# adamkewley/opensim-moco

Measured on AMD Instinct MI355X. Metric: NLP eval_g+eval_jac_g calls/sec (gait10dof18musc), higher is better.
Workload: dtype f64; 1 GPU; MocoTrack gait10dof18musc DGF rigid tendon (configs[2]); mesh_intervals=200, grid_points=401, n=26468, m=20800, nnz_jac=1920800, transcription=hermite-simpson, fd=forward, mode=separate, calls=asynchronous (device pointers, torch stream), parallelism=single

## Files before the change

### opensim-moco_amd/csrc/core.hpp

```cpp
#pragma once
#include <hip/hip_runtime.h>

#include <algorithm>
#include <cmath>
#include <cstdarg>
#include <cstdio>
#include <cstdlib>
#include <cstring>
#include <memory>
#include <string>
#include <type_traits>
#include <vector>

#include "../../include/mocohip.h"
#include "dae_device.hpp"

using namespace mh;

constexpr size_t kMaxLds = 160 * 1024;

typedef __attribute__((address_space(3))) double lds_double;
typedef __attribute__((address_space(3))) int lds_int;
__device__ __forceinline__ lds_double* lds(double* p) { return (lds_double*)p; }

// ... 572 lines not shown
    double* __restrict__ pf;
    const int* __restrict__ tab;
    int nslots;
    int nlc;
    int nl;
    int nq;
    int k0, kshift;
    __device__ __forceinline__ const int* slot(int npc) const { return tab; }
    __device__ __forceinline__ const int* chain(int npc) const { return tab + 2 * npc; }
    __device__ __forceinline__ const int* lane(int npc) const { return tab + 2 * npc + 2 * nslots; }
    __device__ __forceinline__ const int* coord(int npc) const { return lane(npc) + nq; }
    __device__ __forceinline__ const int* bodies(int npc) const { return coord(npc) + nlc; }
    __device__ __forceinline__ long at(int npc, int k, int ln, int e) const {
        return ((long)((k - k0) >> kshift) * nl + ln) * npc + e;
    }
};

struct PathEqs {
    int npc;
    const mh_path_equation* __restrict__ eq;
    const mh_table* __restrict__ tabs;
    const double* __restrict__ brk;
    const double* __restrict__ coef;
    const double* __restrict__ grid;
    FrameDist F;
};

struct EndpointEqs {
    int nep, nnz, W;
    const mh_endpoint_equation* __restrict__ eq;
    const TplEntry* __restrict__ tpl;
};

enum : uint32_t {
    CT_OFF = 0xFFFFFu,
    CT_RAW = 1u << 26,
    CT_GEN = 1u << 27,
    CT_PATH = 1u << 28
};
__device__ __host__ __forceinline__ uint32_t ct_word(uint32_t off, uint32_t coef, uint32_t base) {
    return off | (coef << 20) | (base << 23);
}

__device__ __forceinline__ double div_rn(double a, double b, double y) {
    double q = a * y;
    double r = __builtin_fma(-q, b, a);
    q = __builtin_fma(r, y, q);
    r = __builtin_fma(-q, b, a);
    q = __builtin_fma(r, y, q);
    const double m = __builtin_fabs(a);
    if (!(m >= 0x1p-900 && m <= 0x1p+900) && m != 0.0 && m == m) q = a / b;
    return m == 0.0 ? a * y : q;
}

struct Interval {
    int scheme;
    int interp;
    int ib;
    int rpi;
    int nnz_int;
    int nres;
    int nacc;
    int oaux;
    __device__ __forceinline__ int rout(int r) const { return r < nacc ? r : oaux + (r - nacc); }
    int N;
    int nnz_tail;
    int ntail;
    int npe;
    int nkr;
    int okc;
    PathEqs P;
    EndpointEqs E;
    double* gh;
    double* vh;
    int dbg_stop;
    int pf;
    int qfuse;
    int xcd;
    int dbase;
    uint32_t smagic, sstride, sbase;
    int qdiv;
    const uint32_t* ovl;
    int ov_ne[2], ov_nl[2];
    __device__ __forceinline__ uint32_t base_of(uint32_t w, uint32_t nyall) const {
        const uint32_t off = w & CT_OFF;
        const bool lane = !(w & (CT_GEN | CT_PATH)) && off < nyall;
        return lane ? __umulhi(off, smagic) * sstride + sbase : 0u;
    }
    __device__ __forceinline__ int rows(int i) const { return rpi + (i == N - 1 ? ntail : 0); }
    __device__ __forceinline__ int entries(int i) const { return nnz_int + (i == N - 1 ? nnz_tail : 0); }
};

__device__ __forceinline__ double path_bound(const PathEqs& P, const mh_path_equation& E, double t) {
#pragma clang fp contract(off)
    if (E.table < 0) return E.value;
    const mh_table T = P.tabs[E.table];
    const double* br = P.brk + T.break_begin;
    int s;
    if (t <= br[0]) s = 0;
    else if (t >= br[T.nseg]) s = T.nseg - 1;
    else {
        int lo = 0, hi = T.nseg;
        while (hi - lo > 1) {
            const int mid = (lo + hi) >> 1;
            if (t < br[mid]) hi = mid; else lo = mid;
        }
        s = lo;
    }
    const double* cf = P.coef + T.coef_begin + ((long)s * T.ncol + E.column) * (T.degree + 1);
    const double dt = t - br[s];
    double v = cf[T.degree];
    for (int k = T.degree - 1; k >= 0; --k) v = v * dt + cf[k];
    return v;
}
__device__ __forceinline__ double path_value(const PathEqs& P, int e, double t, double control) {
    const mh_path_equation E = P.eq[e];
    return control - path_bound(P, E, t);
}
__device__ __forceinline__ double path_quot(const PathEqs& P, const Lanes& Ln, int NS, int e, int k,
        double t, double control, int dir) {
#pragma clang fp contract(off)
    const mh_path_equation E = P.eq[e];
    if (dir >= 2 && dir != 2 + NS + E.index) return 0.0;
    const double h = Ln.h;
    double tp = t, tm = t, cp = control, cm = control;
    if (dir < 2) {
        const double g = P.grid[k];
        const double seed = dir == 0 ? 1.0 - g : g;
        tp = t + h * seed;
        tm = t - h * seed;
    } else {
        cp = control + h;
        cm = control - h;
    }
    if (Ln.fd == MH_FD_CENTRAL)
        return ((cp - path_bound(P, E, tp)) - (cm - path_bound(P, E, tm))) / (2.0 * h);
    const double v0 = control - path_bound(P, E, t);
    if (Ln.fd == MH_FD_FORWARD) return ((cp - path_bound(P, E, tp)) - v0) / h;
    return (v0 - (cm - path_bound(P, E, tm))) / h;
}

__device__ __forceinline__ double frame_quot(const PathEqs& P, const Lanes& Ln, int e, int k, int dir) {
#pragma clang fp contract(off)
    const FrameDist& F = P.F;
    if (dir < 2 || dir >= 2 + F.nq) return 0.0;
    const int l = F.lane(P.npc)[dir - 2];
    if (l < 0) return 0.0;
    const double h = Ln.h;
    const double v1 = F.pf[F.at(P.npc, k, 1 + l, e)];
    if (Ln.fd == MH_FD_CENTRAL) return (v1 - F.pf[F.at(P.npc, k, 1 + F.nlc + l, e)]) / (2.0 * h);
    const double v0 = F.pf[F.at(P.npc, k, 0, e)];
    if (Ln.fd == MH_FD_FORWARD) return (v1 - v0) / h;
    return (v0 - v1) / h;
}
template <class YV>
__device__ __forceinline__ double path_row(const PathEqs& P, const YV& Y, int e, int k) {
    const mh_path_equation E = P.eq[e];
    if (E.kind != MH_PATH_CONTROL_BOUND) return P.F.pf[P.F.at(P.npc, k, 0, e)];
    return path_value(P, e, Y.t(k), Y.xc(k, E.index));
}
template <class YV>
__device__ __forceinline__ double path_jac(const PathEqs& P, const Lanes& Ln, int NS, const YV& Y, int e, int k,
        int dir) {
    const mh_path_equation E = P.eq[e];
    if (E.kind != MH_PATH_CONTROL_BOUND) return frame_quot(P, Ln, e, k, dir);
    return path_quot(P, Ln, NS, e, k, Y.t(k), Y.xc(k, E.index), dir);
// ... 186 lines not shown
        if (dir >= 2) {
            v = 0.0 - C.h8 * (dxdot(L, Ln, Y, ki, s, dir) - dxdot(L, Ln, Y, kp, s, dir));
            break;
        }
        const double fi = xdot_at(L, Ln, x, Y, ki, s), fp = xdot_at(L, Ln, x, Y, kp, s);
        v = (dir == 0 ? C.g8 : -C.g8) * (fi - fp) -
            C.h8 * (dxdot(L, Ln, Y, ki, s, dir) - dxdot(L, Ln, Y, kp, s, dir));
        break;
    }
    case T_SIMP_T: {
        const int ki = k_first, km = k_first + 1, kp = k_first + 2;
        if (dir >= 2) {
            v = 0.0 - C.h6 * (dxdot(L, Ln, Y, kp, s, dir) + 4.0 * dxdot(L, Ln, Y, km, s, dir) +
                              dxdot(L, Ln, Y, ki, s, dir));
            break;
        }
        const double fi = xdot_at(L, Ln, x, Y, ki, s), fm = xdot_at(L, Ln, x, Y, km, s),
                     fp = xdot_at(L, Ln, x, Y, kp, s);
        v = (dir == 0 ? C.g6 : -C.g6) * (fp + 4.0 * fm + fi) -
            C.h6 * (dxdot(L, Ln, Y, kp, s, dir) + 4.0 * dxdot(L, Ln, Y, km, s, dir) +
                    dxdot(L, Ln, Y, ki, s, dir));
        break;
    }
    case T_HERM_X: {
        const int k = k_first + T.pt;
        const bool ident = dir == 2 + s;
        if (T.pt == 1) { v = ident ? 1.0 : 0.0; break; }
        if (ident) v += -0.5;
        const double dv = dxdot(L, Ln, Y, k, s, dir);
        v += (T.pt == 0 ? -C.h8 : C.h8) * dv;
        break;
    }
    case T_SIMP_X: {
        const int k = k_first + T.pt;
        const bool ident = dir == 2 + s;
        const double dv = dxdot(L, Ln, Y, k, s, dir);
        if (T.pt == 2) { if (ident) v += 1.0; v += -C.h6 * dv; }
        else if (T.pt == 0) { if (ident) v += -1.0; v += -C.h6 * dv; }
        else v += -C.h6 * 4.0 * dv;
        break;
    }
    case T_INTERP:
        v = T.pt == 1 ? 1.0 : -0.5;
        break;
    case T_RES:
        v = dout(Ln, Y, k_first + T.pt, s, dir);
        break;
    case T_PATH:
        if constexpr (WITH_PATH) {
            const int k = k_first + T.pt;
            v = path_jac(P, Ln, L.NS, Y, s, k, dir);
        }
        break;
    case T_TRAP_T: {
        const int ki = k_first, kp = k_first + 1;
        if (dir >= 2) {
            v = 0.0 - C.hh * (dxdot(L, Ln, Y, kp, s, dir) + dxdot(L, Ln, Y, ki, s, dir));
            break;
        }
        const double fi = xdot_at(L, Ln, x, Y, ki, s), fp = xdot_at(L, Ln, x, Y, kp, s);
        v = (dir == 0 ? C.gh : -C.gh) * (fp + fi) -
            C.hh * (dxdot(L, Ln, Y, kp, s, dir) + dxdot(L, Ln, Y, ki, s, dir));
        break;
    }
    case T_TRAP_X: {
        const int k = k_first + T.pt;
        const bool ident = dir == 2 + s;
        const double dv = dxdot(L, Ln, Y, k, s, dir);
        if (T.pt == 1) { if (ident) v += 1.0; v += -C.hh * dv; }
        else { if (ident) v += -1.0; v += -C.hh * dv; }
        break;
    }
    }
    return v;
}

__device__ __forceinline__ void interval_span(const Interval& I, int i, int& k_first, int& k_last) {
    k_first = grid_of(I, i, 0);
    k_last = k_first + (I.scheme == MH_HERMITE_SIMPSON ? 2 : 1);
}

constexpr int IV_UNROLL = 4;
constexpr int IV_PF = 12;
constexpr int CT_CONST = 4;
constexpr int CT_NCONST = 12;

template <class D, bool GM, bool BASE = false, bool SLDS = false, bool OV = false>
__device__ __forceinline__ void interval_body(const DevModel& M, const Src& S, const Lanes& Ln, const Tasks& TK,
        const Layout& L, const Interval& I, const TplEntry* __restrict__ tpl, const uint32_t* __restrict__ ctpl,
        const int* __restrict__ ctgen, int nctgen,
        const double* __restrict__ T, const double* __restrict__ H, double* __restrict__ g,
        double* __restrict__ values, int il) {
    extern __shared__ double smem[];
    if constexpr (BASE) values = nullptr;
    const int i = I.ib + il;
    int k_first, k_last;
    interval_span(I, i, k_first, k_last);
    const int npts = k_last - k_first + 1;
    const int nt = TK.tdoubles, nh = TK.nmass * D::NST;
    const int ny = D::NO * Ln.stride;
    double* sY = smem;
    double* sTimes = sY + npts * ny;
    double* sK = sTimes + CT_CONST;
    double* sT = sK + CT_NCONST;
    double* sH = sT + (GM ? 0 : npts * nt);
    double* sXs = sH + (GM ? 0 : npts * nh);
    double* sXc = sXs + npts * L.NS;
    double* sXd = sXc + npts * L.NC;
    double* sXm = sXd + npts * L.NDV;
    double* sXl = sXm + npts * L.NM;
    int* sSl = (int*)(sXl + L.NSL);
    const int kl0 = k_first - S.k0;
    if (I.dbg_stop == 7) return;
    if constexpr (BASE && GM) {
        if ((int)threadIdx.x < npts) {
            const int p = threadIdx.x;
            double t;
            const LaneIn<D> in = lane_input<D>(S, Ln, kl0 + p, Ln.base, t);
            sTimes[p] = t;
            const TaskLoadBase<D, const double*> TL{T + (long)(kl0 + p) * nt, H + (long)(kl0 + p) * nh};
            D::combine(M, t, in, TL, LdsOut{lds(sY + p * ny + Ln.base), Ln.stride});
        }
    }
    if (!GM && nt > 0) stage_lds<16>(sT, T + (long)kl0 * nt, npts * nt);
    if (!GM && nh > 0) stage_lds<8>(sH, H + (long)kl0 * nh, npts * nh);
    stage_lds<1>(sXs, S.x + 2 + (long)k_first * L.NS, npts * L.NS);
    if (L.NC > 0) stage_lds<1>(sXc, S.x + 2 + (long)L.NS * L.G + (long)k_first * L.NC, npts * L.NC);
    if (L.NDV > 0)
        stage_lds<1>(sXd, S.x + L.DB + (long)k_first * L.NDV, npts * L.NDV);
    if (L.NM > 0) stage_lds<1>(sXm, S.x + L.XM + (long)k_first * L.NM, npts * L.NM);
    if (L.NSL > 0) stage_lds<1>(sXl, S.x + L.XL + (long)i * L.NSL, L.NSL);
    if constexpr (SLDS)
        for (int q = threadIdx.x; q < Ln.stride * D::NG; q += blockDim.x) sSl[q] = TK.jd[q];
    const double t0 = S.x[0], tf = S.x[1];
    if (threadIdx.x < 2) sK[threadIdx.x] = threadIdx.x ? 1.0 : 0.0;
    __syncthreads();
    if (I.dbg_stop == 1) return;
    using PartAll = std::integral_constant<int, 0>;
    using PartCopies = std::integral_constant<int, 1>;
    using PartSolved = std::integral_constant<int, 2>;
    auto combine_lane = [&](int p, int r, auto partc) {
        constexpr int PART = decltype(partc)::value;
        LaneInL<D> in{lds(sXs + p * L.NS), lds(sXc + p * L.NC), lds(sXd + p * L.NDV), -1, 0.0,
                      lds(sXm + p * L.NM), L.vc(k_first + p) ? lds(sXl) : nullptr};
        const double t = lane_time(Ln, S.grid[k_first + p], t0, tf, r, in.pi, in.step);
        if (PART != 2 && r == Ln.base) sTimes[p] = t;
        const LdsOut out{lds(sY + p * ny + r), Ln.stride};
        auto run = [&](const auto& TL) {
            if constexpr (PART == 1) D::combine_copies(M, t, in, TL, out);
            else if constexpr (PART == 2) D::combine_solved(M, t, in, TL, out);
            else D::combine(M, t, in, TL, out);
        };
        if constexpr (BASE) {
            const TaskLoadBase<D, const lds_double*> TL{lds(sT + p * nt), lds(sH + p * nh)};
            D::combine(M, t, in, TL, out);
        } else if constexpr (GM) {
            const TaskLoadGlobal<D> TL{T + (long)(kl0 + p) * nt, H + (long)(kl0 + p) * nh, TK.jd, r};
            D::combine(M, t, in, TL, out);
        } else if constexpr (SLDS) {
            const TaskLoadLds<D, const lds_int*> TL{lds(sT + p * nt), lds(sH + p * nh), (const lds_int*)sSl, r};
            run(TL);
        } else {
            const TaskLoadLds<D> TL{lds(sT + p * nt), lds(sH + p * nh), TK.jd, r};
            run(TL);
        }
    };
    if constexpr (OV && !BASE && !GM) {
        {
#pragma clang fp contract(off)
            const int B = blockDim.x, tid = threadIdx.x;
            const int nl = npts * Ln.stride;
            const int ncw = (nl + 63) >> 6;
            const int cp = tid / Ln.stride, cr = tid - cp * Ln.stride;
            if (tid < nl) combine_lane(cp, cr, PartCopies{});
            if (tid == B - 1) {
                int pi;
                double st;
                const double ta = lane_time(Ln, S.grid[k_first], t0, tf, Ln.base, pi, st);
                const double tb = lane_time(Ln, S.grid[k_last], t0, tf, Ln.base, pi, st);
                const IvC C0 = iv_const(tb - ta, S.grid[k_last] - S.grid[k_first]);
                sK[2] = 0.0; sK[3] = -C0.h8; sK[4] = C0.h8; sK[5] = -C0.h6; sK[6] = -C0.h6 * 4.0; sK[7] = -C0.hh;
                sK[8] = 0.0; sK[9] = -0.5; sK[10] = 1.0; sK[11] = -1.0;
            }
            __syncthreads();
            double* vi = values + (long)il * I.nnz_int;
            const lds_double* q0 = lds(sY);
            const lds_double* kc = lds(sK + 2);
            const lds_double* kb = lds(sK + 8);
            const int nyall = npts * ny;
            const double h1 = Ln.h, h2 = 2.0 * Ln.h;
            auto run_list = [&](auto fdc, const uint32_t* __restrict__ le, int cap, int n, int j0, int J) {
                constexpr int FD = decltype(fdc)::value;
                const uint32_t* __restrict__ lw = le + cap;
                const uint32_t* __restrict__ lb = lw + cap;
                auto value = [&](uint32_t wu, double q) {
                    const double coef = kc[(wu >> 20) & 7], base = kb[(wu >> 23) & 7];
                    return (wu & CT_RAW) ? q : base + coef * q;
                };
                auto qat = [&](uint32_t off, uint32_t boff) -> double {
                    const double y = q0[off];
                    const bool lane = (int)off < nyall;
                    const double ym = FD == MH_FD_CENTRAL ? q0[lane ? off + Ln.ND : off] : q0[boff];
                    const double qd = FD == MH_FD_CENTRAL ? (y - ym) / h2
                                    : FD == MH_FD_FORWARD ? (y - ym) / h1 : (ym - y) / h1;
                    return lane ? qd : y;
                };
                int j = j0;
                for (; j + (IV_UNROLL - 1) * J < n; j += IV_UNROLL * J) {
                    uint32_t e[IV_UNROLL], w[IV_UNROLL], wb[IV_UNROLL];
                    double q[IV_UNROLL];
#pragma unroll
                    for (int u = 0; u < IV_UNROLL; ++u) {
                        e[u] = le[j + u * J];
                        w[u] = lw[j + u * J];
                        wb[u] = lb[j + u * J];
                    }
#pragma unroll
                    for (int u = 0; u < IV_UNROLL; ++u) q[u] = qat(w[u] & CT_OFF, wb[u]);
#pragma unroll
                    for (int u = 0; u < IV_UNROLL; ++u) vi[e[u]] = value(w[u], q[u]);
                }
                for (; j < n; j += J) {
                    const uint32_t wu = lw[j];
                    vi[le[j]] = value(wu, qat(wu & CT_OFF, lb[j]));
                }
            };
            auto assemble = [&](const uint32_t* le, int cap, int n, int j0, int J) {
                if (Ln.fd == MH_FD_FORWARD) run_list(std::integral_constant<int, MH_FD_FORWARD>{}, le, cap, n, j0, J);
                else if (Ln.fd == MH_FD_BACKWARD)
                    run_list(std::integral_constant<int, MH_FD_BACKWARD>{}, le, cap, n, j0, J);
                else run_list(std::integral_constant<int, MH_FD_CENTRAL>{}, le, cap, n, j0, J);
            };
            const int last = i == I.N - 1;
            if ((tid >> 6) < ncw) {
                if (tid < nl) combine_lane(cp, cr, PartSolved{});
            } else if (I.dbg_stop != 2) {
                assemble(I.ovl, I.ov_ne[1], I.ov_ne[last], tid - ncw * 64, B - ncw * 64);
            }
            __syncthreads();
            if (I.dbg_stop == 2 || I.dbg_stop == 8) return;
            const YS YV{lds(sY), lds(sTimes), D::NO, Ln.stride, k_first, 0, lds(sXs), lds(sXc), L.NS, L.NC,
                        lds(sXd), L.NDV};
            auto g_rows = [&]() {
                if (!g) return;
                double* gi = g + (long)il * I.rpi;
                for (int r = tid; r < I.rows(i); r += B) gi[r] = defect_row(L, I, Ln, S.x, YV, i, r);
            };
            if (I.dbg_stop == 4) { g_rows(); return; }
            assemble(I.ovl + 3 * (long)I.ov_ne[1], I.ov_nl[1], I.ov_nl[last], tid, B);
            const IvC C = iv_const(YV.t(k_last) - YV.t(k_first), S.grid[k_last] - S.grid[k_first]);
            for (int j = tid; j < nctgen; j += B) {
                const int eg = ctgen[j];
                vi[eg] = jac_entry<false>(L, Ln, I.P, S.x, YV, tpl[eg], k_first, C);
            }
            if (I.npe > 0) {
                const int npe = I.npe;
                const int nw = last ? 2 * npe : npe;
                for (int w = tid; w < nw; w += B) {
                    const int ep = w < npe ? w : I.nnz_int + (w - npe);
                    vi[ep] = jac_entry<true>(L, Ln, I.P, S.x, YV, tpl[ep], k_first, C);
                }
            }
            g_rows();
            if (i == 0 && (I.gh || I.vh))
                endpoint_head(L, Ln, I.E, S.x, g ? I.gh : nullptr, I.vh, tid, B);
            return;
        }
    }
    if constexpr (BASE && GM) {
    } else if (BASE || Ln.stride == 1) {
        if ((int)threadIdx.x < npts) combine_lane((int)threadIdx.x, 0, PartAll{});
    } else {
        for (int w = threadIdx.x; w < npts * Ln.stride; w += blockDim.x) {
            const int p = w / Ln.stride, r = w - p * Ln.stride;
            combine_lane(p, r, PartAll{});
        }
    }
    const int ne_iv = values ? I.entries(i) : 0;
    uint32_t pw[IV_PF];
#pragma unroll
    for (int u = 0; u < IV_PF; ++u) {
        const int e = threadIdx.x + u * blockDim.x;
        pw[u] = I.pf && ctpl && e < ne_iv ? ctpl[e] : CT_GEN;
    }
    const uint32_t* __restrict__ cbase = ctpl ? ctpl + I.nnz_int + I.nnz_tail : nullptr;
    uint32_t pb[IV_PF];
#pragma unroll
    for (int u = 0; u < IV_PF; ++u) {
        const int e = threadIdx.x + u * blockDim.x;
        pb[u] = I.pf && ctpl && e < ne_iv ? cbase[e] : 0u;
    }
    int eg0 = -1;
    TplEntry tg0{};
    if (I.pf && ctpl && values && (int)threadIdx.x < nctgen) {
        eg0 = ctgen[threadIdx.x];
        tg0 = tpl[eg0];
    }
    __syncthreads();
    if (values && ctpl && threadIdx.x == 0) {
        const IvC C0 = iv_const(sTimes[npts - 1] - sTimes[0], S.grid[k_last] - S.grid[k_first]);
        sK[2] = 0.0; sK[3] = -C0.h8; sK[4] = C0.h8; sK[5] = -C0.h6; sK[6] = -C0.h6 * 4.0; sK[7] = -C0.hh;
        sK[8] = 0.0; sK[9] = -0.5; sK[10] = 1.0; sK[11] = -1.0;
    }
    if (I.dbg_stop == 2) return;
    const int quot = values && Ln.stride > 1 && !I.qfuse;
    if (quot) {
#pragma clang fp contract(off)
        const int wave = threadIdx.x >> 6, lane = threadIdx.x & 63, nwave = blockDim.x >> 6;
        const double h = Ln.h, h2 = 2.0 * Ln.h;
        for (int po = wave; po < npts * D::NO; po += nwave) {
            lds_double* y = lds(sY + po * Ln.stride);
            const double yb = y[Ln.base];
            for (int d = lane; d < Ln.ND; d += 64) {
                double q;
                if (Ln.fd == MH_FD_CENTRAL) q = (y[d] - y[Ln.ND + d]) / h2;
                else if (Ln.fd == MH_FD_FORWARD) q = (y[d] - yb) / h;
                else q = (yb - y[d]) / h;
                y[d] = q;
            }
        }
        __syncthreads();
    }
    const YS YV{lds(sY), lds(sTimes), D::NO, Ln.stride, k_first, quot, lds(sXs), lds(sXc), L.NS, L.NC,
                lds(sXd), L.NDV};
    if (I.dbg_stop == 3) return;
    if (I.dbg_stop >= 5 && values) {
        double* vi = values + (long)il * I.nnz_int;
        const int ne = I.entries(i);
        double acc = 0.0;
        for (int e = threadIdx.x; e < ne; e += blockDim.x) {
            if (I.dbg_stop == 5) vi[e] = 0.0;
            else {
// ... 673 lines not shown
    std::vector<int> fd_tab;
    size_t fd_lds = 0;
    std::vector<mh_goal> goals;
    std::vector<int32_t> gidx, gcol;
    std::vector<double> gw;
    int nep = 0, nnz_ep = 0;
    int NPAR = 0, NCOPY = 1;
    int64_t XP = 0;
    std::vector<mh_bounds> par_bounds;
    std::vector<mh_parameter_target> par_targets;
    mh_parameter_target* d_par_targets = nullptr;
    std::vector<DevModel> Mp;
    DevModel M0{};
    int* d_lane_main = nullptr;
    int n_lane_main = 0;
    int* d_par_lanes = nullptr;
    int nsprings = 0;
    std::vector<mh_endpoint_equation> ep;
    std::vector<TplEntry> eptpl;
    std::vector<uint8_t> sp_ep;
    EndpointEqs E{};
    double acc_lo = -1000.0, acc_hi = 1000.0;
    int ib = 0, ie = 0, k0 = 0, nk = 0;
    int fd = 0;
    double h = 1e-8;
    int size_class = 0;
    const struct Backend* be = nullptr;
    const struct GenEntry* gen = nullptr;
    Lanes lanes_jac{}, lanes_g{};
    uint64_t model_hash = 0;
    int64_t n = 0, m = 0, nnz = 0;
    std::vector<double> grid, quad;
    std::vector<TplEntry> tpl;
    std::vector<int> tpl_col_pt;
    std::vector<int64_t> tpl_col_off;
    std::vector<mh_variable_info> sinfo, cinfo;
    mh_bounds t_init{}, t_final{};
    int ngoals = 0;
    int device = 0;
    hipStream_t stream = nullptr;
    hipStream_t own_stream = nullptr;
    bool async = false;
    int iv_dbg_stop = 0;
    int iv_pf = 1;
    int iv_dbase = 0;
    std::vector<int> exc_xs;
    bool exc_redirected = false;
    bool exc_full = false;
    uint32_t iv_smagic = 0, iv_sstride = 1, iv_sbase = 0;
    int iv_qdiv = 0;
    int iv_xcd = 1;
    int iv_qfuse = 1;
    hipEvent_t ev[5] = {};
    static constexpr int kMaxD2hChunks = 16;
    int d2h_chunks = 1;
    hipStream_t copy_stream = nullptr;
    hipEvent_t ev_chunk[kMaxD2hChunks] = {};
    hipEvent_t ev_copied = nullptr;
    char* dmem = nullptr;
    DevModel M{};
    GoalSet GS{};
    double* d_quadp = nullptr;
    std::vector<double> quadp;
    double *d_x = nullptr, *d_grid = nullptr, *d_quad = nullptr, *d_times = nullptr, *d_Y = nullptr,
           *d_Yg = nullptr, *d_g = nullptr, *d_vals = nullptr, *d_C = nullptr, *d_grad = nullptr,
           *d_tpart = nullptr, *d_f = nullptr;
    TplEntry* d_tpl = nullptr;
    int* d_exc = nullptr;
    int* d_lane_map = nullptr;
    int n_exc_lanes = 0;
    int* d_exc_slot = nullptr;
    int* d_cmb_map = nullptr;
    int n_exc_gen = 0;
    int g_block = 4;
    bool g_lds = false;
    int g_lds_guard = 0;
    int* d_lds_status = nullptr;
    int groups_split = -1;
    int combine_mode = -1;
    uint32_t* d_ctpl = nullptr;
    std::vector<uint32_t> ctpl;
    int* d_ctgen = nullptr;
    int iv_overlap = 0;
    std::vector<uint32_t> ovl;
    uint32_t* d_ovl = nullptr;
    int ov_ne[2] = {0, 0}, ov_nl[2] = {0, 0};
    std::vector<int> ctgen;
    std::vector<int> rl_e;
    std::vector<uint32_t> rl_w;
    int rl_off[4] = {0, 0, 0, 0}, rl_tail[2] = {0, 0};
    int* d_rl_e = nullptr;
    uint32_t* d_rl_w = nullptr;
    double* d_xch = nullptr;
    double* d_ep = nullptr;
    bool has_marker = false;
    MarkerTrack MT{};
    std::vector<int> mt_tab;
    size_t mt_lds[2] = {0, 0};
    bool use_roles = false;
    int role_threads = 256;
    int iv_threads = 1024;
    int ivg_threads = 256;
    int csplit = 0;
    int ivg_base = 1;
    int ivg_gm = -1;
    int iv_slots_lds = 0;
    bool role_couple = true;
    bool use_ctpl = true;
    float timings[4] = {0, 0, 0, 0};
    TaskSet ts_jac, ts_g, ts_probe;
    bool krec_ok = false;
    KRecs krec_g{};
    double *d_T = nullptr, *d_H = nullptr;
    double *d_Tg = nullptr, *d_Hg = nullptr;
    hipStream_t aux_stream = nullptr;
    hipEvent_t ev_x = nullptr, ev_aux = nullptr;
    const double* x_last = nullptr;
    bool overlap = false;
    char* probe_mem = nullptr;
    double *d_pT = nullptr, *d_pH = nullptr;
    int probe_np = -1;
    struct GraphEntry { int kind; const void *x, *a, *b; hipGraphExec_t exec; };
    std::vector<GraphEntry> graphs;
    bool use_graphs = false;
    bool spin_wait = false;
    bool use_interval[2] = {false, false};
    int nsimd = 1024;
    bool asm_grid_stride = false;
    bool asm_ctpl = true;
    int asm_chunk_ct = 8192;
    bool quot = false;
    const Backend* be_lane = nullptr;
    bool g_lane = false;
    int yq[2] = {0, 0};
    bool timing = false;
    bool groups_timed = false;
    int jac_seeds = 0, nseeds = 0;
    int coloring_order = MH_COLORING_SMALLEST_LAST;
    std::vector<int32_t> seed_color;
    std::vector<int32_t> seed_col_off, seed_cols, seed_ent_off, seed_ents, seed_rows;
    int32_t *d_seed_cols = nullptr, *d_seed_ents = nullptr, *d_seed_rows = nullptr;
    double *d_xp = nullptr, *d_xm = nullptr, *d_gp = nullptr, *d_gm = nullptr;
};

inline Layout make_layout(const mh_ctx* c, int k0, int nk) {
    Layout L{c->NS, c->NC, c->TQ, c->NO, c->NI, c->G, k0, nk, c->NDV, c->NACC, c->SO,
             c->NM, c->NSL, c->OQC, 0, 0, 0};
    L.XM = 2 + (long)(c->NS + c->NC) * c->G;
    L.XL = L.XM + (long)c->NM * c->G;
    L.DB = L.XL + (long)c->NSL * c->N;
    return L;
}

inline Interval make_interval(const mh_ctx* c, double*& g, double*& v) {
    Interval I{c->scheme, c->interp, c->ib, c->rpi, c->nnz_int, c->NMB + c->NAR, c->NMB, c->NQ + c->NZ,
               c->N, c->nnz_tail, c->ntail, c->npe, c->NK, c->OKC, c->P, c->E, nullptr, nullptr, c->iv_dbg_stop, c->iv_pf, c->iv_qfuse,
               c->iv_xcd, c->iv_dbase, c->iv_smagic, c->iv_sstride, c->iv_sbase,
               c->iv_qdiv, c->d_ovl, {c->ov_ne[0], c->ov_ne[1]}, {c->ov_nl[0], c->ov_nl[1]}};
    if (c->ib == 0 && c->nep > 0) {
        I.gh = g;
        I.vh = v;
        if (g) g += c->nep;
        if (v) v += c->nnz_ep;
    }
    return I;
}

inline Src src_of(const mh_ctx* c, const double* x) {
    const Layout L = make_layout(c, c->k0, c->nk);
    return Src{x, c->d_grid, nullptr, c->G, c->k0, L.XM, L.XL, L.DB};
}

int probe_tasks(mh_ctx* c, const TaskInfo& ti, const Lanes& ln, int np);

struct mh_batch {
    std::vector<mh_ctx*> ctx;
    int B = 0;
    BatchItem* d_items = nullptr;
    bool gm = true;
    int waves = 3;
    int threads = 512;
};

struct Backend {
    const char* name;
    void (*eval)(mh_ctx*, const double* x, int mode, double* Y);
    void (*integrand)(mh_ctx*, const double* x);
    void (*grad)(mh_ctx*, const double* x);
    void (*probe)(mh_ctx*, int np, const double* in, double* out);
    double flops_per_eval;
    const TaskInfo* tasks;
    void (*interval)(mh_ctx*, const double* x, int mode, double* g, double* v, int i0, int i1);
    size_t (*interval_bytes)(const mh_ctx*, int mode);
    void (*lanes)(mh_ctx*, const double* x, double* Y);
    void (*batch)(mh_batch*, int mode, const BatchPtrs& P, int with_g, int with_v);
};

template <class D>
static void be_eval_lane(mh_ctx* c, const double* x, int mode, double* Y) {
    Layout L = make_layout(c, c->k0, c->nk);
    const Lanes& ln = mode ? c->lanes_jac : c->lanes_g;
    const long lanes = (long)c->nk * ln.stride;
    const bool exc = mode && c->d_exc && D::EXC_LANES;
    if (mode && c->NPAR > 0) {
        const long nm = (long)c->nk * c->n_lane_main;
        hipLaunchKernelGGL(k_eval<D>, dim3((unsigned)((nm + 63) / 64)), dim3(64), 0, c->stream, c->M, L, ln, x,
                c->d_grid, c->d_times, Y, c->d_lane_main, c->n_lane_main);
        if (exc)
            hipLaunchKernelGGL(k_exc_lanes<D>, dim3((unsigned)((lanes + 63) / 64)), dim3(64), 0, c->stream, c->M,
                    L, ln, x, Y, c->d_exc);
        for (int cp = 1; cp < c->NCOPY; ++cp)
            hipLaunchKernelGGL(k_eval<D>, dim3((unsigned)((c->nk + 63) / 64)), dim3(64), 0, c->stream, c->Mp[cp],
                    L, ln, x, c->d_grid, c->d_times, Y, c->d_par_lanes + (cp - 1), 1);
        return;
    }
    if (!exc) {
        const int tb = (mode == 0 && D::EXC_LANES) ? c->g_block : 64;
        if constexpr (D::EXC_LANES) {
            if (mode == 0 && c->g_lds) {
                const size_t slot = sizeof(typename D::W) + 2 * sizeof(double) * (size_t)c->g_lds_guard;
                const int tl = std::max(1, std::min({tb, 16, (int)(65536 / slot)}));
                const size_t lds = slot * (size_t)tl;
                hipLaunchKernelGGL(k_eval_lds<D>, dim3((unsigned)((lanes + tl - 1) / tl)), dim3(tl), lds,
                        c->stream, c->M, L, ln, x, c->d_grid, c->d_times, Y, c->g_lds_guard, c->d_lds_status);
                return;
            }
        }
        hipLaunchKernelGGL(k_eval<D>, dim3((unsigned)((lanes + tb - 1) / tb)), dim3(tb), 0, c->stream, c->M, L,
                ln, x, c->d_grid, c->d_times, Y, nullptr, 0);
        return;
    }
    const int nmap = ln.stride - c->n_exc_lanes;
    const long full = (long)c->nk * nmap;
    hipLaunchKernelGGL(k_eval<D>, dim3((unsigned)((full + 63) / 64)), dim3(64), 0, c->stream, c->M, L,
            ln, x, c->d_grid, c->d_times, Y, c->d_lane_map, nmap);
    hipLaunchKernelGGL(k_exc_lanes<D>, dim3((unsigned)((lanes + 63) / 64)), dim3(64), 0, c->stream, c->M,
            L, ln, x, Y, c->d_exc);
}
template <class D>
static bool split_groups(const mh_ctx* c) {
    static int decided = -1;
// ... 269 lines not shown
```

### opensim-moco_amd/csrc/mocohip.hip

```cpp
#include "core.hpp"

#include <cstdarg>
#include <limits>

static thread_local std::string g_err;
static int set_err(int code, const char* fmt, ...) {
    char buf[1024];
    va_list ap;
    va_start(ap, fmt);
    vsnprintf(buf, sizeof buf, fmt, ap);
    va_end(ap);
    g_err = buf;
    return code;
}
#define HIPCHK(expr)                                                              \
    do {                                                                          \
        hipError_t e_ = (expr);                                                   \
        if (e_ != hipSuccess)                                                     \
            return set_err(MH_ERR_HIP, "%s failed: %s", #expr, hipGetErrorString(e_)); \
    } while (0)

extern "C" int mh_abi_version(void) { return MH_ABI_VERSION; }
#ifndef MH_BUILD_ID
#define MH_BUILD_ID "unknown"
// ... 2303 lines not shown
        const char* eg = std::getenv("MOCOHIP_GRAPHS");
        c->use_graphs = eg && std::strcmp(eg, "1") == 0;
        const char* es = std::getenv("MOCOHIP_SPIN");
        c->spin_wait = es && std::strcmp(es, "1") == 0;
        const char* ei = std::getenv("MOCOHIP_INTERVAL");
        const bool allow = !(ei && std::strcmp(ei, "0") == 0);
        const char* ec = std::getenv("MOCOHIP_CTPL");
        c->use_ctpl = !(ec && std::strcmp(ec, "0") == 0);
        setup_assembly_variants(c.get());
        const char* er = std::getenv("MOCOHIP_ROLES");
        c->use_roles = er && std::strcmp(er, "1") == 0 && c->NM == 0;
        const char* et = std::getenv("MOCOHIP_ROLE_THREADS");
        if (et) c->role_threads = std::min(512, std::max(64, std::atoi(et) / 64 * 64));
        const char* eqf = std::getenv("MOCOHIP_IV_QFUSE");
        c->iv_qfuse = !(eqf && std::strcmp(eqf, "0") == 0);
        const char* eth = std::getenv("MOCOHIP_IV_THREADS");
        if (eth) c->iv_threads = std::min(1024, std::max(256, std::atoi(eth) / 64 * 64));
        const char* egt = std::getenv("MOCOHIP_IVG_THREADS");
        if (egt) c->ivg_threads = std::min(1024, std::max(64, std::atoi(egt) / 64 * 64));
        const char* eo = std::getenv("MOCOHIP_ROLE_COUPLE");
        c->role_couple = !(eo && std::strcmp(eo, "0") == 0);
        const char* ea = std::getenv("MOCOHIP_ASM");
        c->asm_grid_stride = ea && std::strcmp(ea, "gs") == 0;
        const char* eac = std::getenv("MOCOHIP_ASM_CTPL");
        c->asm_ctpl = !(eac && std::strcmp(eac, "0") == 0);
        if (const char* ech = std::getenv("MOCOHIP_ASM_CHUNK"))
            c->asm_chunk_ct = std::min(1 << 20, std::max(256, std::atoi(ech)));
        const char* ee = std::getenv("MOCOHIP_EVENTS");
        c->timing = ee && std::strcmp(ee, "1") == 0;
        const char* egl = std::getenv("MOCOHIP_G_LANE");
        c->g_lane = egl && std::strcmp(egl, "1") == 0;
        const char* eq = std::getenv("MOCOHIP_QUOT");
        c->quot = eq && std::strcmp(eq, "1") == 0;
        if (redirect_exc_words(c.get()) > 0) {
            setup_assembly_variants(c.get());
            HIPCHK(hipMemcpy(c->d_ctpl, c->ctpl.data(), sizeof(uint32_t) * c->ctpl.size(),
                    hipMemcpyHostToDevice));
        }
        if (o->sparsity_detection != MH_SPARSITY_NONE) {
            const size_t cap = c->tpl.size(), cap_ep = c->eptpl.size();
            int rc2 = detect_sparsity(c.get(), o);
            if (rc2) return rc2;
            c->tpl.clear();
            c->tpl_col_pt.clear();
            build_template(c.get());
            if (!path_entries_lead(c.get()) || c->tpl.size() > cap || c->eptpl.size() > cap_ep)
                return set_err(MH_ERR_INVALID, "internal: detected template layout");
            if (!c->eptpl.empty())
                HIPCHK(hipMemcpy((void*)c->E.tpl, c->eptpl.data(), sizeof(TplEntry) * c->eptpl.size(),
                        hipMemcpyHostToDevice));
            c->E.nnz = c->nnz_ep;
            c->nnz = c->nnz_ep + (int64_t)c->nnz_int * c->N + c->nnz_tail;
            if (!compile_template(c.get())) return set_err(MH_ERR_UNSUPPORTED, "Jacobian template does not compile");
            (void)redirect_exc_words(c.get());
            setup_assembly_variants(c.get());
            HIPCHK(hipMemcpy(c->d_tpl, c->tpl.data(), sizeof(TplEntry) * c->tpl.size(), hipMemcpyHostToDevice));
            HIPCHK(hipMemcpy(c->d_ctpl, c->ctpl.data(), sizeof(uint32_t) * c->ctpl.size(),
                    hipMemcpyHostToDevice));
            if (!c->ctgen.empty())
                HIPCHK(hipMemcpy(c->d_ctgen, c->ctgen.data(), sizeof(int) * c->ctgen.size(),
                        hipMemcpyHostToDevice));
            if (!c->rl_e.empty()) {
                HIPCHK(hipMemcpy(c->d_rl_e, c->rl_e.data(), sizeof(int) * c->rl_e.size(), hipMemcpyHostToDevice));
                HIPCHK(hipMemcpy(c->d_rl_w, c->rl_w.data(), sizeof(uint32_t) * c->rl_w.size(),
                        hipMemcpyHostToDevice));
            }
            c->P.npc = c->npc;
        }
        for (int mode = 0; mode < 2; ++mode)
            c->use_interval[mode] = allow && interval_fits(c.get(), mode);
        const char* eio = std::getenv("MOCOHIP_IV_OVERLAP");
        const int npts_ov = c->scheme == MH_HERMITE_SIMPSON ? 3 : 2;
        const int ncw = (npts_ov * c->lanes_jac.stride + 63) / 64;
        const int ds = c->iv_dbg_stop;
        if (!(eio && std::strcmp(eio, "0") == 0) && tib && c->use_interval[1] && c->use_ctpl && c->iv_qfuse &&
                !c->use_roles && c->lanes_jac.stride > 1 && c->iv_threads > 256 && c->iv_threads / 64 > ncw &&
                ds != 3 && ds != 5 &&
                ds != 6) {
            if (!build_overlap_lists(c.get(), *tib) || c->ovl.size() > ovl_cap)
                return set_err(MH_ERR_INVALID, "internal: k_interval's early entries read a solved output");
            if (!c->ovl.empty())
                HIPCHK(hipMemcpy(c->d_ovl, c->ovl.data(), sizeof(uint32_t) * c->ovl.size(), hipMemcpyHostToDevice));
            c->iv_overlap = 1;
        }
    }
    for (auto& e : c->ev) HIPCHK(hipEventCreate(&e));
    if (const char* ek = std::getenv("MOCOHIP_D2H_CHUNKS"))
        c->d2h_chunks = std::min(mh_ctx::kMaxD2hChunks, std::max(1, std::atoi(ek)));
    HIPCHK(hipStreamCreateWithFlags(&c->aux_stream, hipStreamNonBlocking));
    HIPCHK(hipEventCreateWithFlags(&c->ev_x, hipEventDisableTiming));
    HIPCHK(hipEventCreateWithFlags(&c->ev_aux, hipEventDisableTiming));
    if (const char* eov = std::getenv("MOCOHIP_OVERLAP")) c->overlap = std::strcmp(eov, "1") == 0;
    HIPCHK(hipStreamCreateWithFlags(&c->copy_stream, hipStreamNonBlocking));
    for (auto& e : c->ev_chunk) HIPCHK(hipEventCreateWithFlags(&e, hipEventDisableTiming));
    HIPCHK(hipEventCreateWithFlags(&c->ev_copied, hipEventDisableTiming));
    *out = c.release();
    return MH_OK;
}

extern "C" void mh_destroy(mh_ctx* c) {
    if (!c) return;
    (void)hipSetDevice(c->device);
    if (c->stream) (void)hipStreamSynchronize(c->stream);
    for (auto& e : c->ev)
        if (e) (void)hipEventDestroy(e);
    for (auto& e : c->ev_chunk)
        if (e) (void)hipEventDestroy(e);
    if (c->ev_copied) (void)hipEventDestroy(c->ev_copied);
    if (c->aux_stream) {
        (void)hipStreamSynchronize(c->aux_stream);
        (void)hipStreamDestroy(c->aux_stream);
    }
    if (c->ev_x) (void)hipEventDestroy(c->ev_x);
    if (c->ev_aux) (void)hipEventDestroy(c->ev_aux);
    if (c->copy_stream) {
        (void)hipStreamSynchronize(c->copy_stream);
        (void)hipStreamDestroy(c->copy_stream);
    }
    if (c->own_stream) {
        (void)hipStreamSynchronize(c->own_stream);
        (void)hipStreamDestroy(c->own_stream);
    }
    if (c->dmem) (void)hipFree(c->dmem);
    if (c->probe_mem) (void)hipFree(c->probe_mem);
    for (auto& e : c->graphs) (void)hipGraphExecDestroy(e.exec);
    delete c;
}

extern "C" int mh_get_nlp_info(const mh_ctx* c, mh_nlp_info* info) {
    if (!c || !info) return set_err(MH_ERR_INVALID, "null argument");
    std::memset(info, 0, sizeof *info);
    info->n = c->n;
    info->m = c->m;
    info->nnz_jac_g = c->nnz;
    info->nnz_h_lag = 0;
    info->num_grid_points = c->G;
    info->num_states = c->NS;
    info->num_controls = c->NC;
    info->row_begin = c->ib == 0 ? 0 : c->nep + (int64_t)c->ib * c->rpi;
    info->row_end = c->nep + (int64_t)c->ie * c->rpi + (c->ie == c->N ? c->ntail : 0);
    info->nnz_begin = c->ib == 0 ? 0 : c->nnz_ep + (int64_t)c->ib * c->nnz_int;
    info->nnz_end = c->nnz_ep + (int64_t)c->ie * c->nnz_int + (c->ie == c->N ? c->nnz_tail : 0);
    return MH_OK;
}

static mh_bounds clip(mh_bounds b, mh_bounds e) {
    mh_bounds r;
    r.lower = std::max(b.lower, e.lower);
    r.upper = std::min(b.upper, e.upper);
    return r;
}
static void put_bounds(mh_bounds b, double& lo, double& up) {
    if (!std::isnan(b.lower) && !std::isnan(b.upper)) { lo = b.lower; up = b.upper; }
    else { lo = -INFINITY; up = INFINITY; }
}

extern "C" int mh_get_bounds(const mh_ctx* c, double* xl, double* xu, double* gl, double* gu) {
    if (!c || !xl || !xu) return set_err(MH_ERR_INVALID, "null argument");
    put_bounds(c->t_init, xl[0], xu[0]);
    put_bounds(c->t_final, xl[1], xu[1]);
    auto fill = [&](const mh_variable_info& vi, auto col) {
        const mh_bounds ib = clip(vi.bounds, vi.initial), fb = clip(vi.bounds, vi.final);
        for (int k = 1; k < c->G - 1; ++k) put_bounds(vi.bounds, xl[col(k)], xu[col(k)]);
        put_bounds(ib, xl[col(0)], xu[col(0)]);
        put_bounds(fb, xl[col(c->G - 1)], xu[col(c->G - 1)]);
    };
// ... 1107 lines not shown
    if (flops_per_eval) *flops_per_eval = c->be->flops_per_eval;
    if (model_hash) *model_hash = c->model_hash;
    return MH_OK;
}

extern "C" int mh_get_nlp_info_for(const mh_problem* p, const mh_options* o, mh_nlp_info* info) {
    if (!p || !o || !info) return set_err(MH_ERR_INVALID, "null argument");
    std::unique_ptr<mh_ctx> c(new mh_ctx());
    std::vector<int> coord_body, act_state, ftn_state, mus_control;
    double tau_act, tau_deact;
    int rc = validate_and_layout(c.get(), p, o, coord_body, act_state, ftn_state, mus_control, tau_act,
            tau_deact);
    if (rc) return rc;
    FrameDist FD;
    MarkerTrack MT;
    if ((rc = kinematics_tables(c.get(), p->model, coord_body, FD, MT))) return rc;
    return mh_get_nlp_info(c.get(), info);
}

extern "C" int mh_backend_for(const mh_problem* p, const mh_options* o, char* name, int32_t name_len) {
    if (!p || !o || !name || name_len <= 0) return set_err(MH_ERR_INVALID, "bad argument");
    std::unique_ptr<mh_ctx> c(new mh_ctx());
    std::vector<int> coord_body, act_state, ftn_state, mus_control;
    double tau_act, tau_deact;
    int rc = validate_and_layout(c.get(), p, o, coord_body, act_state, ftn_state, mus_control, tau_act,
            tau_deact);
    if (rc) return rc;
    const Backend* be = select_backend(c.get(), p);
    std::strncpy(name, be->name, (size_t)name_len - 1);
    name[name_len - 1] = 0;
    return MH_OK;
}

extern "C" int mh_debug_interval_overlap(const mh_problem* p, const mh_options* o, int32_t* info8, uint32_t* words,
        uint32_t* bases, uint8_t* early, uint8_t* out_early, int64_t cap) {
    if (!p || !o || !info8) return set_err(MH_ERR_INVALID, "bad argument");
    std::unique_ptr<mh_ctx> c(new mh_ctx());
    std::vector<int> coord_body, act_state, ftn_state, mus_control;
    double tau_act, tau_deact;
    int rc = validate_and_layout(c.get(), p, o, coord_body, act_state, ftn_state, mus_control, tau_act,
            tau_deact);
    if (rc) return rc;
    const Backend* be = select_backend(c.get(), p);
    if (!compile_template(c.get())) return set_err(MH_ERR_UNSUPPORTED, "Jacobian template does not compile");
    const size_t nw = (size_t)c->nnz_int + (size_t)c->nnz_tail;
    const int ND = c->NI + 2 + c->NPAR;
    const int stride = c->fd == MH_FD_CENTRAL ? 2 * ND + 1 : ND + 1;
    const int npts = c->scheme == MH_HERMITE_SIMPSON ? 3 : 2;
    const int32_t info[8] = {(int32_t)nw, c->nnz_int, npts, c->NO, stride, ND, c->fd, stride - 1};
    std::copy(info, info + 8, info8);
    if (cap < (int64_t)nw || cap < c->NO) return MH_OK;
    if (!words || !bases || !early || !out_early) return set_err(MH_ERR_INVALID, "null argument");
    const TaskInfo* ti = be->tasks;
    for (int q = 0; q < c->NO; ++q) out_early[q] = ti && ti->no == c->NO ? ti->out_early[q] : 0;
    std::copy(c->ctpl.begin(), c->ctpl.begin() + nw, words);
    std::copy(c->ctpl.begin() + nw, c->ctpl.begin() + 2 * nw, bases);
    classify_overlap(c->ctpl.data(), nw, npts, c->NO, stride, ND, c->fd, ti && ti->no == c->NO ? ti->out_early : nullptr,
            early);
    return MH_OK;
}

extern "C" int mh_get_callback_sparsity(const mh_ctx* c, uint8_t* pattern, int64_t len) {
    if (!c || !pattern) return set_err(MH_ERR_INVALID, "null argument");
    const size_t W = 1 + (size_t)c->NI, nd = (size_t)c->NO * W, np = nd + (size_t)c->npc * W;
    const size_t need = np + (size_t)c->nep * 2 * W;
    if (len < (int64_t)need) return set_err(MH_ERR_INVALID, "pattern needs %zu bytes", need);
    for (size_t i = 0; i < need; ++i)
        pattern[i] = i < nd ? (c->sp.empty() ? 1 : c->sp[i])
                   : i < np ? (c->sp_pc.empty() ? 1 : c->sp_pc[i - nd])
                            : (c->sp_ep.empty() ? 1 : c->sp_ep[i - np]);
    return MH_OK;
}

extern "C" int mh_get_backend_flags(const mh_ctx* c, char* flags, int32_t len) {
    if (!c || !flags || len <= 0) return set_err(MH_ERR_INVALID, "bad argument");
    std::string f = c->be->tasks ? "tasks" : (std::strncmp(c->be->name, "generic", 7) == 0 ? "generic" : "lane");
    f += c->use_interval[1] ? " interval" : " split";
    if (c->use_interval[0]) f += c->ivg_base ? " interval-g base-slots" : " interval-g";
    if (c->krec_ok) f += " groups-kernarg";
    if (!c->use_ctpl) f += " no-ctpl";
    if (c->iv_dbase) f += " dbase";
    if (c->iv_qdiv) f += " qdiv";
    if (c->use_roles && c->use_interval[1]) f += " roles";
    if (c->iv_overlap && c->use_interval[1]) f += " iv-overlap";
    if (c->quot) f += " quot";
    if (c->asm_grid_stride) f += " asm-gs";
    if (c->d_exc) f += " exc-lanes";
    if (c->d_exc_slot)
        f += c->exc_redirected && c->use_ctpl && c->asm_ctpl && !c->asm_grid_stride ? " exc-fill adot-only"
                                                                                     : " exc-fill";
    if (c->g_lds && !c->be->tasks && std::strncmp(c->be->name, "generic", 7) == 0) {
        f += " g-lds";
        if (c->g_lds_guard) {
            int st = 0;
            if (hipMemcpyAsync(&st, c->d_lds_status, sizeof(int), hipMemcpyDeviceToHost, c->stream) != hipSuccess ||
                    hipStreamSynchronize(c->stream) != hipSuccess)
                return set_err(MH_ERR_HIP, "reading the LDS guard status failed");
            f += st ? " g-lds-guard-violated" : " g-lds-guard-intact";
        }
    }
    std::strncpy(flags, f.c_str(), (size_t)len - 1);
    flags[len - 1] = 0;
    return MH_OK;
}

extern "C" int mh_get_work(const mh_ctx* c, double* work4) {
    if (!c || !work4) return set_err(MH_ERR_INVALID, "null argument");
    const double lanes_jac = (double)c->nk * c->lanes_jac.stride, lanes_g = (double)c->nk;
    if (c->be->tasks) {
        work4[0] = c->ts_jac.flops;
        work4[1] = c->ts_g.flops;
        work4[2] = c->ts_jac.ntasks;
    } else {
        work4[0] = lanes_jac * c->be->flops_per_eval;
        work4[1] = lanes_g * c->be->flops_per_eval;
        work4[2] = 0.0;
    }
    work4[3] = lanes_jac;
    return MH_OK;
}

static const Backend* select_backend(mh_ctx* c, const mh_problem* p) {
    c->model_hash = model_hash(&p->model);
    const char* force = std::getenv("MOCOHIP_BACKEND");
    const bool generic = force && std::strcmp(force, "generic") == 0;
    const bool lane = force && std::strcmp(force, "lane") == 0;
    if (!generic && c->NPAR == 0 && c->nsprings == 0) {
        for (auto entry : kGeneratedModels) {
            const GenEntry& e = entry();
            if (e.implicit != (c->NMB > 0) || e.prescribed != (c->presc != 0)) continue;
            if (c->NKC && !c->presc && (e.kc_enforce != (c->enforce != 0) || e.kc_slacks != (c->NSL > 0)))
                continue;
            if (!e.match(p->model)) continue;
            c->gen = &e;
            c->be_lane = &e.lane;
            return lane ? &e.lane : &e.tasks;
        }
    }
    return &generic_backends()[c->size_class];
}
```

Measured before the change: 26300 calls/s.

## Software-pipeline overlap-list index loads in interval Jacobian assembly

Adds a pipelined assembly path for the overlapped interval kernel. Index triples for the early list are loaded before LDS staging. The next batch of indices is prefetched while the current batch is computed. Late-list indices are loaded ahead by the combine warps before the barrier, and the time-step constants are computed earlier. The aim is to hide global-memory latency on index fetches, at the cost of more registers (IvBatch copies) and added code complexity, with an env var to turn it off.

```diff
diff --git a/opensim-moco_amd/csrc/core.hpp b/opensim-moco_amd/csrc/core.hpp
--- a/opensim-moco_amd/csrc/core.hpp
+++ b/opensim-moco_amd/csrc/core.hpp
@@ -678,6 +678,7 @@
     int qdiv;
     const uint32_t* ovl;
     int ov_ne[2], ov_nl[2];
+    int pipe;
     __device__ __forceinline__ uint32_t base_of(uint32_t w, uint32_t nyall) const {
         const uint32_t off = w & CT_OFF;
         const bool lane = !(w & (CT_GEN | CT_PATH)) && off < nyall;
@@ -1030,6 +1031,14 @@
 
 constexpr int IV_UNROLL = 4;
 constexpr int IV_PF = 12;
+constexpr int IVP_BATCH = 1;
+constexpr int IVP_EARLY = 2;
+constexpr int IVP_LATE = 4;
+constexpr int IVP_CONST = 8;
+constexpr int IVP_DEFAULT = IVP_BATCH | IVP_EARLY | IVP_LATE | IVP_CONST;
+struct IvBatch {
+    uint32_t e[IV_UNROLL], w[IV_UNROLL], wb[IV_UNROLL];
+};
 constexpr int CT_CONST = 4;
 constexpr int CT_NCONST = 12;
 
@@ -1060,6 +1069,35 @@
     int* sSl = (int*)(sXl + L.NSL);
     const int kl0 = k_first - S.k0;
     if (I.dbg_stop == 7) return;
+    auto iv_load = [&](IvBatch& b, uint32_t off, int cap, int n, int j, int J) {
+#pragma unroll
+        for (int u = 0; u < IV_UNROLL; ++u) {
+            const int ju = j + u * J;
+            const bool ok = ju < n;
+            const uint32_t o = ok ? off + (uint32_t)ju : 0u, c = ok ? (uint32_t)cap : 0u;
+            b.e[u] = I.ovl[o];
+            b.w[u] = I.ovl[o + c];
+            b.wb[u] = I.ovl[o + 2u * c];
+        }
+    };
+    const int ivp = I.pipe;
+    IvBatch ovb;
+    if constexpr (OV && !BASE && !GM) {
+        const int B = blockDim.x, tid = threadIdx.x;
+        const int ncw = (npts * Ln.stride + 63) >> 6;
+        if ((ivp & IVP_EARLY) && (tid >> 6) >= ncw && I.dbg_stop != 2)
+            iv_load(ovb, 0u, I.ov_ne[1], I.ov_ne[i == I.N - 1], tid - ncw * 64, B - ncw * 64);
+        if ((ivp & IVP_CONST) && tid == B - 1) {
+#pragma clang fp contract(off)
+            int pi;
+            double st;
+            const double ta = lane_time(Ln, S.grid[k_first], S.x[0], S.x[1], Ln.base, pi, st);
+            const double tb = lane_time(Ln, S.grid[k_last], S.x[0], S.x[1], Ln.base, pi, st);
+            const IvC C0 = iv_const(tb - ta, S.grid[k_last] - S.grid[k_first]);
+            sK[2] = 0.0; sK[3] = -C0.h8; sK[4] = C0.h8; sK[5] = -C0.h6; sK[6] = -C0.h6 * 4.0; sK[7] = -C0.hh;
+            sK[8] = 0.0; sK[9] = -0.5; sK[10] = 1.0; sK[11] = -1.0;
+        }
+    }
     if constexpr (BASE && GM) {
         if ((int)threadIdx.x < npts) {
             const int p = threadIdx.x;
@@ -1121,7 +1159,7 @@
             const int ncw = (nl + 63) >> 6;
             const int cp = tid / Ln.stride, cr = tid - cp * Ln.stride;
             if (tid < nl) combine_lane(cp, cr, PartCopies{});
-            if (tid == B - 1) {
+            if (!(ivp & IVP_CONST) && tid == B - 1) {
                 int pi;
                 double st;
                 const double ta = lane_time(Ln, S.grid[k_first], t0, tf, Ln.base, pi, st);
@@ -1137,22 +1175,61 @@
             const lds_double* kb = lds(sK + 8);
             const int nyall = npts * ny;
             const double h1 = Ln.h, h2 = 2.0 * Ln.h;
+            auto value = [&](uint32_t wu, double q) {
+                const double coef = kc[(wu >> 20) & 7], base = kb[(wu >> 23) & 7];
+                return (wu & CT_RAW) ? q : base + coef * q;
+            };
+            auto quot_at = [&](auto fdc, uint32_t off, uint32_t boff) -> double {
+                constexpr int FD = decltype(fdc)::value;
+                const double y = q0[off];
+                const bool lane = (int)off < nyall;
+                const double ym = FD == MH_FD_CENTRAL ? q0[lane ? off + Ln.ND : off] : q0[boff];
+                const double qd = FD == MH_FD_CENTRAL ? (y - ym) / h2
+                                : FD == MH_FD_FORWARD ? (y - ym) / h1 : (ym - y) / h1;
+                return lane ? qd : y;
+            };
+            const int last = i == I.N - 1;
+            const uint32_t loff = 3u * (uint32_t)I.ov_ne[1];
+            const int ne = I.ov_ne[last], nla = I.ov_nl[last];
+            auto run_pipe = [&](auto fdc, IvBatch& cur, uint32_t off, int cap, int n, int j0, int J, bool then_late) {
+                for (int j = j0; j < n;) {
+                    const int jn = j + IV_UNROLL * J;
+                    const bool more = jn < n;
+                    IvBatch nxt = cur;
+                    if (then_late)
+                        iv_load(nxt, more ? off : loff, more ? cap : I.ov_nl[1], more ? n : nla, more ? jn : tid,
+                                more ? J : B);
+                    else if (more) iv_load(nxt, off, cap, n, jn, J);
+                    double q[IV_UNROLL];
+#pragma unroll
+                    for (int u = 0; u < IV_UNROLL; ++u) {
+                        const bool ok = j + u * J < n;
+                        q[u] = quot_at(fdc, ok ? cur.w[u] & CT_OFF : 0u, ok ? cur.wb[u] : 0u);
+                    }
+                    double v[IV_UNROLL];
+#pragma unroll
+                    for (int u = 0; u < IV_UNROLL; ++u) v[u] = value(j + u * J < n ? cur.w[u] : 0u, q[u]);
+#pragma unroll
+                    for (int u = 0; u < IV_UNROLL; ++u) asm volatile("" : "+v"(v[u]));
+#pragma unroll
+                    for (int u = 0; u < IV_UNROLL; ++u)
+                        if (j + u * J < n) vi[cur.e[u]] = v[u];
+                    cur = nxt;
+                    j = jn;
+                }
+                if (then_late && j0 >= n) iv_load(cur, loff, I.ov_nl[1], nla, tid, B);
+            };
+            auto assemble_pipe = [&](IvBatch& cur, uint32_t off, int cap, int n, int j0, int J, bool then_late) {
+                if (Ln.fd == MH_FD_FORWARD)
+                    run_pipe(std::integral_constant<int, MH_FD_FORWARD>{}, cur, off, cap, n, j0, J, then_late);
+                else if (Ln.fd == MH_FD_BACKWARD)
+                    run_pipe(std::integral_constant<int, MH_FD_BACKWARD>{}, cur, off, cap, n, j0, J, then_late);
+                else run_pipe(std::integral_constant<int, MH_FD_CENTRAL>{}, cur, off, cap, n, j0, J, then_late);
+            };
             auto run_list = [&](auto fdc, const uint32_t* __restrict__ le, int cap, int n, int j0, int J) {
-                constexpr int FD = decltype(fdc)::value;
                 const uint32_t* __restrict__ lw = le + cap;
                 const uint32_t* __restrict__ lb = lw + cap;
-                auto value = [&](uint32_t wu, double q) {
-                    const double coef = kc[(wu >> 20) & 7], base = kb[(wu >> 23) & 7];
-                    return (wu & CT_RAW) ? q : base + coef * q;
-                };
-                auto qat = [&](uint32_t off, uint32_t boff) -> double {
-                    const double y = q0[off];
-                    const bool lane = (int)off < nyall;
-                    const double ym = FD == MH_FD_CENTRAL ? q0[lane ? off + Ln.ND : off] : q0[boff];
-                    const double qd = FD == MH_FD_CENTRAL ? (y - ym) / h2
-                                    : FD == MH_FD_FORWARD ? (y - ym) / h1 : (ym - y) / h1;
-                    return lane ? qd : y;
-                };
+                auto qat = [&](uint32_t off, uint32_t boff) -> double { return quot_at(fdc, off, boff); };
                 int j = j0;
                 for (; j + (IV_UNROLL - 1) * J < n; j += IV_UNROLL * J) {
                     uint32_t e[IV_UNROLL], w[IV_UNROLL], wb[IV_UNROLL];
@@ -1179,11 +1256,20 @@
                     run_list(std::integral_constant<int, MH_FD_BACKWARD>{}, le, cap, n, j0, J);
                 else run_list(std::integral_constant<int, MH_FD_CENTRAL>{}, le, cap, n, j0, J);
             };
-            const int last = i == I.N - 1;
+            const bool batch = ivp & IVP_BATCH, late_ahead = batch && (ivp & IVP_LATE);
+            IvBatch ovt;
             if ((tid >> 6) < ncw) {
                 if (tid < nl) combine_lane(cp, cr, PartSolved{});
+                if (late_ahead && I.dbg_stop != 2) iv_load(ovt, loff, I.ov_nl[1], nla, tid, B);
             } else if (I.dbg_stop != 2) {
-                assemble(I.ovl, I.ov_ne[1], I.ov_ne[last], tid - ncw * 64, B - ncw * 64);
+                if (batch) {
+                    const int j0 = tid - ncw * 64, J = B - ncw * 64;
+                    if (!(ivp & IVP_EARLY)) iv_load(ovb, 0u, I.ov_ne[1], ne, j0, J);
+                    assemble_pipe(ovb, 0u, I.ov_ne[1], ne, j0, J, late_ahead);
+                    if (late_ahead) ovt = ovb;
+                } else {
+                    assemble(I.ovl, I.ov_ne[1], ne, tid - ncw * 64, B - ncw * 64);
+                }
             }
             __syncthreads();
             if (I.dbg_stop == 2 || I.dbg_stop == 8) return;
@@ -1195,7 +1281,12 @@
                 for (int r = tid; r < I.rows(i); r += B) gi[r] = defect_row(L, I, Ln, S.x, YV, i, r);
             };
             if (I.dbg_stop == 4) { g_rows(); return; }
-            assemble(I.ovl + 3 * (long)I.ov_ne[1], I.ov_nl[1], I.ov_nl[last], tid, B);
+            if (batch) {
+                if (!late_ahead) iv_load(ovt, loff, I.ov_nl[1], nla, tid, B);
+                assemble_pipe(ovt, loff, I.ov_nl[1], nla, tid, B, false);
+            } else {
+                assemble(I.ovl + 3 * (long)I.ov_ne[1], I.ov_nl[1], nla, tid, B);
+            }
             const IvC C = iv_const(YV.t(k_last) - YV.t(k_first), S.grid[k_last] - S.grid[k_first]);
             for (int j = tid; j < nctgen; j += B) {
                 const int eg = ctgen[j];
@@ -2035,6 +2126,7 @@
     std::vector<uint32_t> ctpl;
     int* d_ctgen = nullptr;
     int iv_overlap = 0;
+    int iv_pipe = 0;
     std::vector<uint32_t> ovl;
     uint32_t* d_ovl = nullptr;
     int ov_ne[2] = {0, 0}, ov_nl[2] = {0, 0};
@@ -2109,7 +2201,7 @@
     Interval I{c->scheme, c->interp, c->ib, c->rpi, c->nnz_int, c->NMB + c->NAR, c->NMB, c->NQ + c->NZ,
                c->N, c->nnz_tail, c->ntail, c->npe, c->NK, c->OKC, c->P, c->E, nullptr, nullptr, c->iv_dbg_stop, c->iv_pf, c->iv_qfuse,
                c->iv_xcd, c->iv_dbase, c->iv_smagic, c->iv_sstride, c->iv_sbase,
-               c->iv_qdiv, c->d_ovl, {c->ov_ne[0], c->ov_ne[1]}, {c->ov_nl[0], c->ov_nl[1]}};
+               c->iv_qdiv, c->d_ovl, {c->ov_ne[0], c->ov_ne[1]}, {c->ov_nl[0], c->ov_nl[1]}, c->iv_pipe};
     if (c->ib == 0 && c->nep > 0) {
         I.gh = g;
         I.vh = v;
diff --git a/opensim-moco_amd/csrc/mocohip.hip b/opensim-moco_amd/csrc/mocohip.hip
--- a/opensim-moco_amd/csrc/mocohip.hip
+++ b/opensim-moco_amd/csrc/mocohip.hip
@@ -2409,6 +2409,9 @@
             if (!c->ovl.empty())
                 HIPCHK(hipMemcpy(c->d_ovl, c->ovl.data(), sizeof(uint32_t) * c->ovl.size(), hipMemcpyHostToDevice));
             c->iv_overlap = 1;
+            const char* eip = std::getenv("MOCOHIP_IV_PIPE");
+            c->iv_pipe = eip ? (std::atoi(eip) & IVP_DEFAULT) : IVP_DEFAULT;
+            if (!(c->iv_pipe & IVP_BATCH)) c->iv_pipe &= IVP_CONST;
         }
     }
     for (auto& e : c->ev) HIPCHK(hipEventCreate(&e));
@@ -3682,7 +3685,7 @@
     if (c->iv_dbase) f += " dbase";
     if (c->iv_qdiv) f += " qdiv";
     if (c->use_roles && c->use_interval[1]) f += " roles";
-    if (c->iv_overlap && c->use_interval[1]) f += " iv-overlap";
+    if (c->iv_overlap && c->use_interval[1]) f += c->iv_pipe ? " iv-overlap iv-pipe" : " iv-overlap";
     if (c->quot) f += " quot";
     if (c->asm_grid_stride) f += " asm-gs";
     if (c->d_exc) f += " exc-lanes";
```

Measured after the change: 25710 calls/s. 0.978x the previous value.
